# AshishKumar4/FlaxDiff

Measured on AMD Instinct MI355X. Metric: train images/sec/node (64x64 uncond EDM UNet, bs=256), higher is better.
Workload: dtype bf16; 1 GPU; model=unet_64px_[64,128,256,512]_res2_heads4, global_batch=256, resolution=64, parallelism=dp1, schedule=EDM + KarrasPredictionTransform(sigma_data=0.5)

## Files before the change

### flaxdiff_amd/ops/hip/conv2d_halo_v2.hip

```cpp
#include <torch/extension.h>
#include <ATen/hip/HIPContext.h>
#include "common.h"
#include "host_util.h"

typedef __bf16 bf16v8h __attribute__((ext_vector_type(8)));

#define HV2_NTH 256
#define HV2_BK 64

union HBF8 { bf16v8h v; ushort u[8]; uint4 q; };

__device__ __forceinline__ void hv2_glds16(const ushort* src, ushort* dst) {
    __builtin_amdgcn_global_load_lds(
        (const __attribute__((address_space(1))) void*)src,
        (__attribute__((address_space(3))) void*)dst, 16, 0, 0);
}

struct HaloEpilogue {
    float4 bs[2][2][2];
    uint4 av[2][2][2], bv[2][2][2];

    __device__ __forceinline__ void load_bias(const float* __restrict__ bias,
                                              const int nl) {
        #pragma unroll
        for (int fn = 0; fn < 2; ++fn) {
            #pragma unroll
            for (int p = 0; p < 2; ++p) {
                const float4* b = reinterpret_cast<const float4*>(
                    bias + nl + fn * 32 + p * 16);
                bs[fn][p][0] = b[0];
                bs[fn][p][1] = b[1];
            }
        }
    }

    __device__ __forceinline__ void load_adds(const ushort* __restrict__ addp,
                                              const ushort* __restrict__ baddp,
                                              const long m0, const int nl,
                                              const long RW, const int Cout,
                                              const long M) {
        #pragma unroll
        for (int fm = 0; fm < 2; ++fm) {
            const long m = m0 + fm * 32;
            const long mc = m < M ? m : M - 1;
            if (addp) {
                const ushort* a = addp + mc * Cout + nl;
                #pragma unroll
                for (int fn = 0; fn < 2; ++fn) {
                    #pragma unroll
                    for (int p = 0; p < 2; ++p)
                        av[fm][fn][p] = *reinterpret_cast<const uint4*>(
                            a + fn * 32 + p * 16);
                }
            }
            if (baddp) {
                const ushort* b = baddp
                    + (long)((unsigned)mc / (unsigned)RW) * Cout + nl;
                #pragma unroll
                for (int fn = 0; fn < 2; ++fn) {
                    #pragma unroll
                    for (int p = 0; p < 2; ++p)
                        bv[fm][fn][p] = *reinterpret_cast<const uint4*>(
                            b + fn * 32 + p * 16);
                }
            }
        }
    }

    static __device__ __forceinline__ void add_bf8(float (&v)[8], const uint4 u) {
        const uint w[4] = {u.x, u.y, u.z, u.w};
        #pragma unroll
        for (int i = 0; i < 4; ++i) {
            v[2 * i] += __uint_as_float(w[i] << 16);
            v[2 * i + 1] += __uint_as_float(w[i] & 0xffff0000u);
        }
    }

    __device__ __forceinline__ void finish(const f32x16 (&acc)[2][2],
                                           const bool has_bias,
                                           const bool has_add,
                                           const bool has_badd,
                                           ushort* __restrict__ Y,
                                           const long m0, const int nl,
                                           const int Cout, const long M) const {
        #pragma unroll
        for (int fm = 0; fm < 2; ++fm) {
            const long m = m0 + fm * 32;
            ushort* yrow = Y + m * Cout + nl;
            #pragma unroll
            for (int fn = 0; fn < 2; ++fn) {
                #pragma unroll
                for (int p = 0; p < 2; ++p) {
                    float v[8];
                    #pragma unroll
                    for (int j = 0; j < 4; ++j) {
                        const auto r = __builtin_amdgcn_permlane32_swap(
                            __float_as_uint(acc[fn][fm][(2 * p) * 4 + j]),
                            __float_as_uint(acc[fn][fm][(2 * p + 1) * 4 + j]),
                            false, false);
                        v[j] = __uint_as_float(r[0]);
                        v[4 + j] = __uint_as_float(r[1]);
                    }
                    if (has_bias) {
                        const float4 b0 = bs[fn][p][0], b1 = bs[fn][p][1];
                        v[0] += b0.x; v[1] += b0.y; v[2] += b0.z; v[3] += b0.w;
                        v[4] += b1.x; v[5] += b1.y; v[6] += b1.z; v[7] += b1.w;
                    }
                    if (has_add) add_bf8(v, av[fm][fn][p]);
                    if (has_badd) add_bf8(v, bv[fm][fn][p]);
                    uint4 pk;
                    pk.x = f2bf(v[0]) | ((uint)f2bf(v[1]) << 16);
                    pk.y = f2bf(v[2]) | ((uint)f2bf(v[3]) << 16);
                    pk.z = f2bf(v[4]) | ((uint)f2bf(v[5]) << 16);
                    pk.w = f2bf(v[6]) | ((uint)f2bf(v[7]) << 16);
                    if (m < M)
                        *reinterpret_cast<uint4*>(yrow + fn * 32 + p * 16) = pk;
                }
            }
        }
    }
};

template <bool TRANSPOSED, int BMT, int BNT, int W, bool UP = false>
__global__ __launch_bounds__(HV2_NTH, 2)
void conv2d_halo_v2_kernel(
        const ushort* __restrict__ X,
        const ushort* __restrict__ Wt,
        const float* __restrict__ bias,
        const ushort* __restrict__ addp,
        const ushort* __restrict__ baddp,
        ushort* __restrict__ Y,
        const int Bn, const int R,
        const int Cin, const int Cout,
        const long M) {
    constexpr int RPT = BMT / W;
    constexpr int NSLOT = RPT + 2;
    constexpr int NROW_H = NSLOT * (W + 2);
    constexpr int ZR = NROW_H;
    constexpr int WB0 = NROW_H + 3;
    constexpr int NW = BNT / 32;
    constexpr int NHC = (NSLOT * W / 8 + 3) / 4;
    constexpr int WMW = BMT / 64;

    extern __shared__ __attribute__((aligned(16))) ushort hlds[];
    const int tid = threadIdx.x;
    const int lane = tid & 63;
    const int wid = tid >> 6;
    const int wn = wid / WMW;
    const int wm = wid % WMW;
    const int half = lane >> 5;
    const int l31 = lane & 31;

    const long m_base = (long)blockIdx.x * BMT;
    const int n_base = blockIdx.y * BNT;
    const long grow0 = m_base / W;
    const long BH = (long)Bn * R;
    const int ksl = Cin / HV2_BK;

    const int n_wave = n_base + wn * 64;
    const bool wave_live = n_wave < Cout;
    const int nl = n_wave + half * 8;
    const long m0 = m_base + wm * 64 + l31;
    HaloEpilogue epi;
    if (bias && wave_live) epi.load_bias(bias, nl);

    auto issue_halo = [&](int ci0) {
        #pragma unroll
        for (int i = 0; i < NHC; ++i) {
            int q = wid + i * 4;
            const int qmax = NSLOT * W / 8 - 1;
            q = q > qmax ? qmax : q;
            const int slot = q / (W / 8);
            const int c = q % (W / 8);
            long g = grow0 + slot - 1;
            g = g < 0 ? 0 : (g >= BH ? BH - 1 : g);
            const int pos0 = c * 8;
            const int rowbase = slot * (W + 2) + 1 + pos0;
            const int pix = pos0 + (lane >> 3);
            const int key = (rowbase + (lane >> 3)) & 7;
            const ushort* s;
            if (UP) {
                const int b = (int)(g / R);
                const int r = (int)(g - (long)b * R);
                const long gs = (long)b * (R >> 1) + (r >> 1);
                s = X + (gs * (W >> 1) + (pix >> 1)) * (long)Cin + ci0
                  + (((lane & 7) ^ key) << 3);
            } else {
                s = X + (g * W + pix) * (long)Cin + ci0
                  + (((lane & 7) ^ key) << 3);
            }
            hv2_glds16(s, hlds + rowbase * 64);
        }
    };
    auto issue_w = [&](int flat) {
        const int tap = flat % 9;
        const int ci0 = (flat / 9) * HV2_BK;
        const ushort* wslab = Wt + (long)tap * Cout * Cin;
        const int buf = (WB0 + (flat % 3) * BNT) * 64;
        #pragma unroll
        for (int i = 0; i < NW; ++i) {
            const int row0 = (wid + i * 4) * 8;
            const int r8 = lane >> 3;
            const int key = ((row0 + r8) & 7);
            int co = n_base + row0 + r8;
            co = co < Cout ? co : Cout - 1;
            const ushort* s = wslab + (long)co * Cin + ci0
                            + (((lane & 7) ^ key) << 3);
            hv2_glds16(s, hlds + buf + row0 * 64);
        }
    };

    f32x16 acc[2][2] = {};
    const int nflat = 9 * ksl;

    issue_halo(0);
    issue_w(0);
    issue_w(1);

    for (int i = tid; i < 3 * 64; i += HV2_NTH)
        hlds[ZR * 64 + i] = 0;
    for (int i = tid; i < NSLOT * 2 * 64; i += HV2_NTH) {
        const int sl = i >> 7;
        const int e = (i >> 6) & 1;
        hlds[(sl * (W + 2) + (e ? (W + 1) : 0)) * 64 + (i & 63)] = 0;
    }

    int brow[2][3];
    #pragma unroll
    for (int fm = 0; fm < 2; ++fm) {
        const long m = m0 + fm * 32;
        const unsigned mc = (unsigned)(m < M ? m : M - 1);
        const int ow = (int)(mc % W);
        const unsigned grow = mc / W;
        const int orow = (int)(grow % (unsigned)R);
        #pragma unroll
        for (int dr = -1; dr <= 1; ++dr) {
            if (m >= M || orow + dr < 0 || orow + dr >= R) {
                brow[fm][dr + 1] = ZR + 1;
            } else {
                const int slot = (int)(grow - (unsigned)grow0) + dr + 1;
                brow[fm][dr + 1] = slot * (W + 2) + ow + 1;
            }
        }
    }

    auto tap_step = [&](const int flat, const bool last) {
        const int tap = flat % 9;
        const int sci = flat / 9;
        if (last || (tap == 0 && sci > 0)) {
            asm volatile("s_waitcnt vmcnt(0) lgkmcnt(0)" ::: "memory");
        } else {
            asm volatile("s_waitcnt vmcnt(%0) lgkmcnt(0)" :: "i"(NW) : "memory");
        }
        __builtin_amdgcn_s_barrier();
        if (last) {
            if (wave_live)
                epi.load_adds(addp, baddp, m0, nl, (long)R * W, Cout, M);
        } else if (flat + 2 < nflat) {
            issue_w(flat + 2);
        }

        const int r = tap / 3, s = tap % 3;
        const int dr = TRANSPOSED ? (1 - r) : (r - 1);
        const int ds = TRANSPOSED ? (1 - s) : (s - 1);
        const int wbuf = (WB0 + (flat % 3) * BNT) * 64;
        const int ar0 = wn * 64 + l31;
        const int ar1 = ar0 + 32;
        const int br0 = brow[0][dr + 1] + ds;
        const int br1 = brow[1][dr + 1] + ds;
        #pragma unroll
        for (int kk = 0; kk < HV2_BK / 16; ++kk) {
            const int k0 = kk * 16 + half * 8;
            const int ch = k0 >> 3;
            bf16v8h a0 = reinterpret_cast<const HBF8*>(
                hlds + wbuf + ar0 * 64 + ((ch ^ (ar0 & 7)) << 3))->v;
            bf16v8h a1 = reinterpret_cast<const HBF8*>(
                hlds + wbuf + ar1 * 64 + ((ch ^ (ar1 & 7)) << 3))->v;
            bf16v8h b0 = reinterpret_cast<const HBF8*>(
                hlds + br0 * 64 + ((ch ^ (br0 & 7)) << 3))->v;
            bf16v8h b1 = reinterpret_cast<const HBF8*>(
                hlds + br1 * 64 + ((ch ^ (br1 & 7)) << 3))->v;
            acc[0][0] = __builtin_amdgcn_mfma_f32_32x32x16_bf16(a0, b0, acc[0][0], 0, 0, 0);
            acc[0][1] = __builtin_amdgcn_mfma_f32_32x32x16_bf16(a0, b1, acc[0][1], 0, 0, 0);
            acc[1][0] = __builtin_amdgcn_mfma_f32_32x32x16_bf16(a1, b0, acc[1][0], 0, 0, 0);
            acc[1][1] = __builtin_amdgcn_mfma_f32_32x32x16_bf16(a1, b1, acc[1][1], 0, 0, 0);
        }
        if (!last && tap == 8) {
            __builtin_amdgcn_s_barrier();
            issue_halo((sci + 1) * HV2_BK);
        }
    };
    for (int flat = 0; flat < nflat - 1; ++flat)
        tap_step(flat, false);
    tap_step(nflat - 1, true);

    if (wave_live)
        epi.finish(acc, bias != nullptr, addp != nullptr, baddp != nullptr,
                   Y, m0, nl, Cout, M);
}

template <int BMT, int BNT, int W>
static size_t hv2_smem() {
    constexpr int NROW = (BMT / W + 2) * (W + 2) + 3 + 3 * BNT;
    return (size_t)NROW * 64 * sizeof(ushort);
}

bool conv2d_halo_v2_launch(const void* x, const void* wt, const float* bias,
                           const ushort* addp, const ushort* baddp,
                           void* y, bool transposed,
                           int B, int R, int W, int Cin, int Cout, long M,
                           hipStream_t stream, bool upsample) {
    FD_FLUSH_STALE();
    if (Cin % 64 || Cout % 64) return false;
    if (M >= (1L << 31)) return false;
    if (W != 8 && W != 16 && W != 32 && W != 64) return false;
    int bmt = (Cout <= 64) ? 256 : 128;
    static const bool w64_256tile = std::getenv("FD_HALO_W64_128TILE") == nullptr;
    if (bmt == 128 && W == 64) {
        if (!w64_256tile) {
            if (Cin / HV2_BK < 2) return false;
        } else {
            bmt = 256;
        }
    }
    const int bnt = 128 * 128 / bmt;
    if (bmt % W) return false;
    if (M % W) return false;

    if (upsample && ((R & 1) || (W & 1))) return false;

    dim3 grid((unsigned)((M + bmt - 1) / bmt), (unsigned)((Cout + bnt - 1) / bnt));
    const int mode = upsample ? 2 : (transposed ? 1 : 0);
    #define HV2_KEY(MODE_, BMT_, W_) (((MODE_) << 16) | ((BMT_) << 7) | (W_))
    #define HV2_CASE(MODE_, BMT_, W_)                                          \
        case HV2_KEY(MODE_, BMT_, W_):                                         \
            fd_launch_lds<conv2d_halo_v2_kernel<(MODE_ == 1), BMT_,            \
                                                128 * 128 / BMT_, W_,          \
                                                (MODE_ == 2)>>(                \
                grid, dim3(HV2_NTH), hv2_smem<BMT_, 128 * 128 / BMT_, W_>(),   \
                stream, (const ushort*)x, (const ushort*)wt, bias, addp,       \
                baddp, (ushort*)y, B, R, Cin, Cout, M);                        \
            break;
    #define HV2_TILE(MODE_, BMT_)                                              \
        HV2_CASE(MODE_, BMT_, 8) HV2_CASE(MODE_, BMT_, 16)                     \
        HV2_CASE(MODE_, BMT_, 32) HV2_CASE(MODE_, BMT_, 64)
    switch (HV2_KEY(mode, bmt, W)) {
        HV2_TILE(0, 128) HV2_TILE(0, 256)
        HV2_TILE(1, 128) HV2_TILE(1, 256)
        HV2_TILE(2, 128) HV2_TILE(2, 256)
        default: return false;
    }
    #undef HV2_TILE
    #undef HV2_CASE
    #undef HV2_KEY
    FD_CHECK_LAUNCH();
    return true;
}
```

### flaxdiff_amd/ops/hip/gemm_bf16.hip

```cpp
#include <torch/extension.h>
#include <ATen/hip/HIPContext.h>
#include "common.h"
#include "host_util.h"

typedef __bf16 bf16v8m __attribute__((ext_vector_type(8)));
typedef __attribute__((__vector_size__(4 * sizeof(__bf16)))) __bf16 bf16x4m;

#define GM_NTH 256
#define GM_BK 64

union MBF8 { bf16v8m v; ushort u[8]; uint4 q; ushort4 h4[2]; };

__device__ __forceinline__ void gm_glds16(const ushort* src, ushort* dst) {
    __builtin_amdgcn_global_load_lds(
        (const __attribute__((address_space(1))) void*)src,
        (__attribute__((address_space(3))) void*)dst, 16, 0, 0);
}

__device__ __forceinline__ bf16x4m gm_tr(const ushort* p) {
    return __builtin_amdgcn_ds_read_tr16_b64_v4bf16(
        (__attribute__((address_space(3))) bf16x4m*)p);
}

template <bool BT, int BMT, int BNT, int LOOK, bool XSPLIT = false>
__global__ __launch_bounds__(GM_NTH, 2)
void gemm_bf16_kernel(const ushort* __restrict__ X,
                      const ushort* __restrict__ W,
                      const float* __restrict__ bias,
                      const ushort* __restrict__ addp,
                      ushort* __restrict__ Y,
                      const long M, const int N, const int K,
                      const long mt_lo_stride,
                      const ushort* __restrict__ X2,
                      const int Ka) {
    constexpr int WMW = BMT / 64;
    constexpr int XTILE = BMT * GM_BK;
    constexpr int KP = (BNT == 128) ? 68 : 64;
    constexpr int WTILE = BT ? (BNT * GM_BK) : ((BNT / 16) * KP * 16);
    constexpr int DBUF = LOOK + 1;
    constexpr int NGX = BMT / 32;
    constexpr int NGW = BNT / 32;
    constexpr int NG = NGX + NGW;

    extern __shared__ __attribute__((aligned(16))) ushort gmlds[];
    ushort* Xr = gmlds;
    ushort* Wr = gmlds + DBUF * XTILE;

    const int tid = threadIdx.x;
    const int lane = tid & 63;
    const int wid = tid >> 6;
    const int wn = wid / WMW;
    const int wm = wid % WMW;
    const int half = lane >> 5;
    const int l31 = lane & 31;
    const int n_base = blockIdx.y * BNT;
    const int ksl = K / GM_BK;

    const long mt0 = (long)blockIdx.x * mt_lo_stride;
    const long mtiles = (M + BMT - 1) / BMT;
    const long mt1 = (mt0 + mt_lo_stride < mtiles) ? mt0 + mt_lo_stride : mtiles;
    const int nsteps = (int)(mt1 - mt0) * ksl;
    if (nsteps <= 0) return;

    auto issue = [&](int f) {
        const int fc = f >= nsteps ? nsteps - 1 : f;
        const long mb = (mt0 + fc / ksl) * BMT;
        const int k0 = (fc % ksl) * GM_BK;
        const int buf = fc % DBUF;
        ushort* xd = Xr + buf * XTILE;
        const ushort* xs = X + k0;
        int xstride = K;
        if (XSPLIT) {
            const bool second = k0 >= Ka;
            xs = second ? X2 + (k0 - Ka) : X + k0;
            xstride = second ? K - Ka : Ka;
        }
        #pragma unroll
        for (int i = 0; i < NGX; ++i) {
            const int row0 = (wid + i * 4) * 8;
            const int r8 = lane >> 3;
            long m = mb + row0 + r8;
            m = m < M ? m : M - 1;
            const int key = (row0 + r8) & 7;
            gm_glds16(xs + m * xstride + (((lane & 7) ^ key) << 3),
                      xd + row0 * GM_BK);
        }
        ushort* wd = Wr + buf * WTILE;
        if (BT) {
            #pragma unroll
            for (int i = 0; i < NGW; ++i) {
                const int row0 = (wid + i * 4) * 8;
                const int r8 = lane >> 3;
                int n = n_base + row0 + r8;
                n = n < N ? n : N - 1;
                const int key = (row0 + r8) & 7;
                gm_glds16(W + (long)n * K + k0 + (((lane & 7) ^ key) << 3),
                          wd + row0 * GM_BK);
            }
        } else {
            #pragma unroll
            for (int i = 0; i < NGW; ++i) {
                const int pi = wid + i * 4;
                const int p = pi >> 1;
                const int kr0 = (pi & 1) * 32;
                int nc = n_base + p * 16 + (lane & 1) * 8;
                if (nc + 8 > N) nc = N - 8;
                gm_glds16(W + (long)(k0 + kr0 + (lane >> 1)) * N + nc,
                          wd + p * KP * 16 + kr0 * 16);
            }
        }
    };

    #pragma unroll
    for (int l = 0; l < LOOK; ++l) issue(l);

    const int ltr = ((lane >> 4) & 1) * KP * 16 + ((lane >> 5) << 3) * 16
                  + (lane & 15) * 4;

    constexpr int NFN = 2;
    f32x16 acc[NFN][2] = {};

    long cur_mt = mt0;
    for (int f = 0; f < nsteps; ++f) {
        asm volatile("s_waitcnt vmcnt(%0)" :: "i"((LOOK - 1) * NG) : "memory");
        __builtin_amdgcn_s_barrier();
        issue(f + LOOK);
        const int buf = f % DBUF;
        const ushort* Xb = Xr + buf * XTILE;
        const ushort* Wb = Wr + buf * WTILE;

        #pragma unroll
        for (int kk = 0; kk < GM_BK / 16; ++kk) {
            const int k0 = kk * 16 + half * 8;
            const int ch = k0 >> 3;
            MBF8 a0, a1;
            if (BT) {
                const int ar0 = wn * 64 + l31;
                a0 = *reinterpret_cast<const MBF8*>(
                    Wb + ar0 * GM_BK + ((ch ^ (ar0 & 7)) << 3));
                if (NFN == 2) {
                    const int ar1 = ar0 + 32;
                    a1 = *reinterpret_cast<const MBF8*>(
                        Wb + ar1 * GM_BK + ((ch ^ (ar1 & 7)) << 3));
                }
            } else {
                const ushort* ap = Wb + wn * 4 * KP * 16 + ltr + kk * 16 * 16;
                bf16x4m t0 = gm_tr(ap), t1 = gm_tr(ap + 64);
                a0.h4[0] = *reinterpret_cast<ushort4*>(&t0);
                a0.h4[1] = *reinterpret_cast<ushort4*>(&t1);
                if (NFN == 2) {
                    const ushort* ap2 = ap + 2 * KP * 16;
                    bf16x4m t2 = gm_tr(ap2), t3 = gm_tr(ap2 + 64);
                    a1.h4[0] = *reinterpret_cast<ushort4*>(&t2);
                    a1.h4[1] = *reinterpret_cast<ushort4*>(&t3);
                }
            }
            const int br0 = wm * 64 + l31;
            const int br1 = br0 + 32;
            const bf16v8m b0 = reinterpret_cast<const MBF8*>(
                Xb + br0 * GM_BK + ((ch ^ (br0 & 7)) << 3))->v;
            const bf16v8m b1 = reinterpret_cast<const MBF8*>(
                Xb + br1 * GM_BK + ((ch ^ (br1 & 7)) << 3))->v;
            acc[0][0] = __builtin_amdgcn_mfma_f32_32x32x16_bf16(a0.v, b0, acc[0][0], 0, 0, 0);
            acc[0][1] = __builtin_amdgcn_mfma_f32_32x32x16_bf16(a0.v, b1, acc[0][1], 0, 0, 0);
            if (NFN == 2) {
                acc[1][0] = __builtin_amdgcn_mfma_f32_32x32x16_bf16(a1.v, b0, acc[1][0], 0, 0, 0);
                acc[1][1] = __builtin_amdgcn_mfma_f32_32x32x16_bf16(a1.v, b1, acc[1][1], 0, 0, 0);
            }
        }

        if ((f % ksl) == ksl - 1) {
            const long m_base = cur_mt * BMT;
            #pragma unroll
            for (int fm = 0; fm < 2; ++fm) {
                const long m = m_base + wm * 64 + fm * 32 + l31;
                if (m < M) {
                    ushort* yrow = Y + m * N;
                    #pragma unroll
                    for (int fn = 0; fn < NFN; ++fn) {
                        #pragma unroll
                        for (int qq = 0; qq < 4; ++qq) {
                            const int n0 = n_base + wn * 64 + fn * 32 + qq * 8
                                         + half * 4;
                            if (n0 >= N) continue;
                            float v0 = acc[fn][fm][qq * 4 + 0];
                            float v1 = acc[fn][fm][qq * 4 + 1];
                            float v2 = acc[fn][fm][qq * 4 + 2];
                            float v3 = acc[fn][fm][qq * 4 + 3];
                            if (bias) {
                                v0 += bias[n0];
                                v1 += (n0 + 1 < N) ? bias[n0 + 1] : 0.f;
                                v2 += (n0 + 2 < N) ? bias[n0 + 2] : 0.f;
                                v3 += (n0 + 3 < N) ? bias[n0 + 3] : 0.f;
                            }
                            if (addp && n0 + 4 <= N) {
                                const ushort4 av = *reinterpret_cast<
                                    const ushort4*>(addp + m * N + n0);
                                v0 += bf2f(av.x); v1 += bf2f(av.y);
                                v2 += bf2f(av.z); v3 += bf2f(av.w);
                            } else if (addp) {
                                for (int j = 0; j < 4 && n0 + j < N; ++j) {
                                    const float av = bf2f(addp[m * N + n0 + j]);
                                    if (j == 0) v0 += av;
                                    else if (j == 1) v1 += av;
                                    else if (j == 2) v2 += av;
                                    else v3 += av;
                                }
                            }
                            if (n0 + 4 <= N) {
                                ushort4 pk;
                                pk.x = f2bf(v0); pk.y = f2bf(v1);
                                pk.z = f2bf(v2); pk.w = f2bf(v3);
                                *reinterpret_cast<ushort4*>(yrow + n0) = pk;
                            } else {
                                const float vs[4] = {v0, v1, v2, v3};
                                for (int j = 0; j < 4 && n0 + j < N; ++j)
                                    yrow[n0 + j] = f2bf(vs[j]);
                            }
                        }
                    }
                }
            }
            #pragma unroll
            for (int a = 0; a < NFN; ++a) {
                acc[a][0] = (f32x16){};
                acc[a][1] = (f32x16){};
            }
            ++cur_mt;
        }
    }
    asm volatile("s_waitcnt vmcnt(0)" ::: "memory");
}

torch::Tensor gemm_fwd(torch::Tensor x, torch::Tensor w, torch::Tensor bias) {
    FD_FLUSH_STALE();
    TORCH_CHECK(x.is_cuda() && x.is_contiguous() && w.is_contiguous());
    TORCH_CHECK(x.scalar_type() == at::kBFloat16 && w.scalar_type() == at::kBFloat16);
    const long M = x.size(0);
    const int K = x.size(1), N = w.size(1);
    TORCH_CHECK(w.size(0) == K && K % GM_BK == 0);
    auto y = torch::empty({M, (long)N}, x.options());
    const float* bias_ptr = nullptr;
    torch::Tensor bias_f;
    if (bias.defined() && bias.numel()) {
        bias_f = bias.to(at::kFloat).contiguous();
        bias_ptr = bias_f.data_ptr<float>();
    }
    const int bmt = (N <= 64) ? 256 : 128;
    const int bnt = 128 * 128 / bmt;
    const long mtiles = (M + bmt - 1) / bmt;
    const int ntiles = (N + bnt - 1) / bnt;
    long bm = std::max<long>(1, std::min<long>(mtiles, 768 / std::max(1, ntiles)));
    const long tpb = (mtiles + bm - 1) / bm;
    bm = (mtiles + tpb - 1) / tpb;
    auto stream = at::hip::getCurrentHIPStream();
    dim3 grid((unsigned)bm, (unsigned)ntiles);
    if (bmt == 256) {
        constexpr size_t smem = 2 * (256 * 64 + 4 * 64 * 16) * sizeof(ushort);
        fd_launch_lds<gemm_bf16_kernel<false, 256, 64, 1>>(grid, dim3(GM_NTH), smem, stream,
                           (const ushort*)x.data_ptr(), (const ushort*)w.data_ptr(),
                           bias_ptr, nullptr, (ushort*)y.data_ptr(), M, N, K, tpb,
                           (const ushort*)nullptr, 0);
    } else {
        constexpr size_t smem = 2 * (128 * 64 + 8 * 68 * 16) * sizeof(ushort);
        fd_launch_lds<gemm_bf16_kernel<false, 128, 128, 1>>(grid, dim3(GM_NTH), smem, stream,
                           (const ushort*)x.data_ptr(), (const ushort*)w.data_ptr(),
                           bias_ptr, nullptr, (ushort*)y.data_ptr(), M, N, K, tpb,
                           (const ushort*)nullptr, 0);
    }
    FD_CHECK_LAUNCH();
    return y;
}

torch::Tensor gemm_dx(torch::Tensor dy, torch::Tensor w) {
    FD_FLUSH_STALE();
    TORCH_CHECK(dy.is_cuda() && dy.is_contiguous() && w.is_contiguous());
    const long M = dy.size(0);
    const int N = dy.size(1), K = w.size(0);
    TORCH_CHECK(w.size(1) == N && N % GM_BK == 0);
    auto dx = torch::empty({M, (long)K}, dy.options());
    const int bmt = (K <= 64) ? 256 : 128;
    const int bnt = 128 * 128 / bmt;
    const long mtiles = (M + bmt - 1) / bmt;
    const int ntiles = (K + bnt - 1) / bnt;
    long bm = std::max<long>(1, std::min<long>(mtiles, 768 / std::max(1, ntiles)));
    const long tpb = (mtiles + bm - 1) / bm;
    bm = (mtiles + tpb - 1) / tpb;
    auto stream = at::hip::getCurrentHIPStream();
    dim3 grid((unsigned)bm, (unsigned)ntiles);
    if (bmt == 256) {
        constexpr size_t smem = 2 * (256 * 64 + 64 * 64) * sizeof(ushort);
        fd_launch_lds<gemm_bf16_kernel<true, 256, 64, 1>>(grid, dim3(GM_NTH), smem, stream,
                           (const ushort*)dy.data_ptr(), (const ushort*)w.data_ptr(),
                           nullptr, nullptr, (ushort*)dx.data_ptr(), M, K, N, tpb,
                           (const ushort*)nullptr, 0);
    } else {
        constexpr size_t smem = 2 * (128 * 64 + 128 * 64) * sizeof(ushort);
        fd_launch_lds<gemm_bf16_kernel<true, 128, 128, 1>>(grid, dim3(GM_NTH), smem, stream,
                           (const ushort*)dy.data_ptr(), (const ushort*)w.data_ptr(),
                           nullptr, nullptr, (ushort*)dx.data_ptr(), M, K, N, tpb,
                           (const ushort*)nullptr, 0);
    }
    FD_CHECK_LAUNCH();
    return dx;
}

torch::Tensor gemm_nt(torch::Tensor x, torch::Tensor wt, torch::Tensor bias,
                      torch::Tensor addt, c10::optional<torch::Tensor> x2) {
    FD_FLUSH_STALE();
    TORCH_CHECK(x.is_cuda() && x.is_contiguous() && wt.is_contiguous());
    const long M = x.size(0);
    const bool split = fd_has(x2);
    const int Ka = x.size(1);
    const ushort* x2_ptr = nullptr;
    if (split) {
        TORCH_CHECK(x2->is_cuda() && x2->device() == x.device() &&
                    x2->is_contiguous() && x2->dim() == 2 && x2->size(0) == M &&
                    x2->scalar_type() == at::kBFloat16 &&
                    x.scalar_type() == at::kBFloat16 &&
                    Ka % GM_BK == 0 && x2->size(1) % GM_BK == 0,
                    "gemm_nt: x2 must be bf16 [M, Kb] with Ka, Kb % 64 == 0");
        x2_ptr = (const ushort*)x2->data_ptr();
    }
    const int K = Ka + (split ? (int)x2->size(1) : 0), N = wt.size(0);
    TORCH_CHECK(wt.size(1) == K && K % GM_BK == 0);
    auto y = torch::empty({M, (long)N}, x.options());
    const float* bias_ptr = nullptr;
    torch::Tensor bias_f;
    if (bias.defined() && bias.numel()) {
        bias_f = bias.to(at::kFloat).contiguous();
        bias_ptr = bias_f.data_ptr<float>();
    }
    const ushort* add_ptr = nullptr;
    if (addt.defined() && addt.numel()) {
        TORCH_CHECK(addt.is_contiguous() && addt.numel() == M * N &&
                    addt.scalar_type() == at::kBFloat16,
                    "gemm_nt add tensor must be bf16 [M, N]");
        add_ptr = (const ushort*)addt.data_ptr();
    }
    const int bmt = (N <= 64) ? 256 : 128;
    const int bnt = 128 * 128 / bmt;
    const long mtiles = (M + bmt - 1) / bmt;
    const int ntiles = (N + bnt - 1) / bnt;
    long bm = std::max<long>(1, std::min<long>(mtiles, 768 / std::max(1, ntiles)));
    const long tpb = (mtiles + bm - 1) / bm;
    bm = (mtiles + tpb - 1) / tpb;
    auto stream = at::hip::getCurrentHIPStream();
    dim3 grid((unsigned)bm, (unsigned)ntiles);
    #define GM_NT_LAUNCH(BMT_, BNT_, SPLIT_)                                   \
        fd_launch_lds<gemm_bf16_kernel<true, BMT_, BNT_, 1, SPLIT_>>(          \
            grid, dim3(GM_NTH),                                                \
            (size_t)2 * (BMT_ * 64 + BNT_ * 64) * sizeof(ushort), stream,      \
            (const ushort*)x.data_ptr(), (const ushort*)wt.data_ptr(),         \
            bias_ptr, add_ptr, (ushort*)y.data_ptr(), M, N, K, tpb,            \
            x2_ptr, Ka)
    if (bmt == 256) {
        if (split) GM_NT_LAUNCH(256, 64, true);
        else GM_NT_LAUNCH(256, 64, false);
    } else {
        if (split) GM_NT_LAUNCH(128, 128, true);
        else GM_NT_LAUNCH(128, 128, false);
    }
    #undef GM_NT_LAUNCH
    FD_CHECK_LAUNCH();
    return y;
}

__global__ void transpose_shadows_kernel(const ushort* __restrict__ src_base,
                                         ushort* __restrict__ dst_base,
                                         const int* __restrict__ tiles,
                                         const int ntiles2) {
    __shared__ ushort tsm[64][65];
    for (int t = blockIdx.x; t < ntiles2; t += gridDim.x) {
        const int* rec = tiles + (long)t * 4;
        const long soff = (unsigned)rec[0];
        const long doff = (unsigned)rec[1];
        const int N = rec[2];
        const int K = rec[3];
        const int lane = threadIdx.x & 63;
        const int w = threadIdx.x >> 6;
        __syncthreads();
        #pragma unroll
        for (int r = 0; r < 16; ++r) {
            const int row = w * 16 + r;
            tsm[row][lane] = src_base[soff + (long)row * N + lane];
        }
        __syncthreads();
        #pragma unroll
        for (int r = 0; r < 16; ++r) {
            const int row = w * 16 + r;
            dst_base[doff + (long)row * K + lane] = tsm[lane][row];
        }
    }
}

void transpose_shadows(torch::Tensor src_flat, torch::Tensor dst_flat,
                       torch::Tensor tiles) {
    FD_FLUSH_STALE();
    TORCH_CHECK(src_flat.is_cuda() && tiles.scalar_type() == at::kInt);
    const int n = tiles.size(0);
    if (!n) return;
    auto stream = at::hip::getCurrentHIPStream();
    const int blocks = std::min(n, 2048);
    hipLaunchKernelGGL(transpose_shadows_kernel, dim3(blocks), dim3(256), 0,
                       stream, (const ushort*)src_flat.data_ptr(),
                       (ushort*)dst_flat.data_ptr(), tiles.data_ptr<int>(), n);
    FD_CHECK_LAUNCH();
}
```

Baseline: 6230 images/s.

## Unify LDS swizzle keys with compile-time conflict proofs and share the vectorized MFMA epilogue

Moves the XOR chunk swizzle into a shared lds_swizzle header. The halo conv now adds a per-slot key delta so B-fragment reads across halo rows avoid LDS bank conflicts, and constexpr static_asserts check that reads stay conflict-free for each tile shape and width. The GEMM kernel gains a FAST template path that reuses the halo conv's permlane-based epilogue, with bias preloaded and add tensors prefetched before the final k-step, so stores are 16-byte vectorized. This adds register pressure for the prefetched epilogue data and more template variants to compile.

Result: faster. 6381 images/s, median of 6 (+2.4%).

```diff
diff --git a/flaxdiff_amd/ops/hip/conv2d_halo_v2.hip b/flaxdiff_amd/ops/hip/conv2d_halo_v2.hip
--- a/flaxdiff_amd/ops/hip/conv2d_halo_v2.hip
+++ b/flaxdiff_amd/ops/hip/conv2d_halo_v2.hip
@@ -2,6 +2,8 @@
 #include <ATen/hip/HIPContext.h>
 #include "common.h"
 #include "host_util.h"
+#include "lds_swizzle.h"
+#include "mfma_epilogue.h"
 
 typedef __bf16 bf16v8h __attribute__((ext_vector_type(8)));
 
@@ -15,111 +17,6 @@
         (const __attribute__((address_space(1))) void*)src,
         (__attribute__((address_space(3))) void*)dst, 16, 0, 0);
 }
-
-struct HaloEpilogue {
-    float4 bs[2][2][2];
-    uint4 av[2][2][2], bv[2][2][2];
-
-    __device__ __forceinline__ void load_bias(const float* __restrict__ bias,
-                                              const int nl) {
-        #pragma unroll
-        for (int fn = 0; fn < 2; ++fn) {
-            #pragma unroll
-            for (int p = 0; p < 2; ++p) {
-                const float4* b = reinterpret_cast<const float4*>(
-                    bias + nl + fn * 32 + p * 16);
-                bs[fn][p][0] = b[0];
-                bs[fn][p][1] = b[1];
-            }
-        }
-    }
-
-    __device__ __forceinline__ void load_adds(const ushort* __restrict__ addp,
-                                              const ushort* __restrict__ baddp,
-                                              const long m0, const int nl,
-                                              const long RW, const int Cout,
-                                              const long M) {
-        #pragma unroll
-        for (int fm = 0; fm < 2; ++fm) {
-            const long m = m0 + fm * 32;
-            const long mc = m < M ? m : M - 1;
-            if (addp) {
-                const ushort* a = addp + mc * Cout + nl;
-                #pragma unroll
-                for (int fn = 0; fn < 2; ++fn) {
-                    #pragma unroll
-                    for (int p = 0; p < 2; ++p)
-                        av[fm][fn][p] = *reinterpret_cast<const uint4*>(
-                            a + fn * 32 + p * 16);
-                }
-            }
-            if (baddp) {
-                const ushort* b = baddp
-                    + (long)((unsigned)mc / (unsigned)RW) * Cout + nl;
-                #pragma unroll
-                for (int fn = 0; fn < 2; ++fn) {
-                    #pragma unroll
-                    for (int p = 0; p < 2; ++p)
-                        bv[fm][fn][p] = *reinterpret_cast<const uint4*>(
-                            b + fn * 32 + p * 16);
-                }
-            }
-        }
-    }
-
-    static __device__ __forceinline__ void add_bf8(float (&v)[8], const uint4 u) {
-        const uint w[4] = {u.x, u.y, u.z, u.w};
-        #pragma unroll
-        for (int i = 0; i < 4; ++i) {
-            v[2 * i] += __uint_as_float(w[i] << 16);
-            v[2 * i + 1] += __uint_as_float(w[i] & 0xffff0000u);
-        }
-    }
-
-    __device__ __forceinline__ void finish(const f32x16 (&acc)[2][2],
-                                           const bool has_bias,
-                                           const bool has_add,
-                                           const bool has_badd,
-                                           ushort* __restrict__ Y,
-                                           const long m0, const int nl,
-                                           const int Cout, const long M) const {
-        #pragma unroll
-        for (int fm = 0; fm < 2; ++fm) {
-            const long m = m0 + fm * 32;
-            ushort* yrow = Y + m * Cout + nl;
-            #pragma unroll
-            for (int fn = 0; fn < 2; ++fn) {
-                #pragma unroll
-                for (int p = 0; p < 2; ++p) {
-                    float v[8];
-                    #pragma unroll
-                    for (int j = 0; j < 4; ++j) {
-                        const auto r = __builtin_amdgcn_permlane32_swap(
-                            __float_as_uint(acc[fn][fm][(2 * p) * 4 + j]),
-                            __float_as_uint(acc[fn][fm][(2 * p + 1) * 4 + j]),
-                            false, false);
-                        v[j] = __uint_as_float(r[0]);
-                        v[4 + j] = __uint_as_float(r[1]);
-                    }
-                    if (has_bias) {
-                        const float4 b0 = bs[fn][p][0], b1 = bs[fn][p][1];
-                        v[0] += b0.x; v[1] += b0.y; v[2] += b0.z; v[3] += b0.w;
-                        v[4] += b1.x; v[5] += b1.y; v[6] += b1.z; v[7] += b1.w;
-                    }
-                    if (has_add) add_bf8(v, av[fm][fn][p]);
-                    if (has_badd) add_bf8(v, bv[fm][fn][p]);
-                    uint4 pk;
-                    pk.x = f2bf(v[0]) | ((uint)f2bf(v[1]) << 16);
-                    pk.y = f2bf(v[2]) | ((uint)f2bf(v[3]) << 16);
-                    pk.z = f2bf(v[4]) | ((uint)f2bf(v[5]) << 16);
-                    pk.w = f2bf(v[6]) | ((uint)f2bf(v[7]) << 16);
-                    if (m < M)
-                        *reinterpret_cast<uint4*>(yrow + fn * 32 + p * 16) = pk;
-                }
-            }
-        }
-    }
-};
 
 template <bool TRANSPOSED, int BMT, int BNT, int W, bool UP = false>
 __global__ __launch_bounds__(HV2_NTH, 2)
@@ -177,7 +74,8 @@
             const int pos0 = c * 8;
             const int rowbase = slot * (W + 2) + 1 + pos0;
             const int pix = pos0 + (lane >> 3);
-            const int key = (rowbase + (lane >> 3)) & 7;
+            const int key = lds_swz::chunk_key(
+                rowbase + (lane >> 3) + lds_swz::halo_key_delta(W) * slot);
             const ushort* s;
             if (UP) {
                 const int b = (int)(g / R);
@@ -201,7 +99,7 @@
         for (int i = 0; i < NW; ++i) {
             const int row0 = (wid + i * 4) * 8;
             const int r8 = lane >> 3;
-            const int key = ((row0 + r8) & 7);
+            const int key = lds_swz::chunk_key(row0 + r8);
             int co = n_base + row0 + r8;
             co = co < Cout ? co : Cout - 1;
             const ushort* s = wslab + (long)co * Cin + ci0
@@ -226,6 +124,7 @@
     }
 
     int brow[2][3];
+    int kd[2];
     #pragma unroll
     for (int fm = 0; fm < 2; ++fm) {
         const long m = m0 + fm * 32;
@@ -233,6 +132,7 @@
         const int ow = (int)(mc % W);
         const unsigned grow = mc / W;
         const int orow = (int)(grow % (unsigned)R);
+        kd[fm] = lds_swz::halo_key_delta(W) * ((int)(grow - (unsigned)grow0) + 1);
         #pragma unroll
         for (int dr = -1; dr <= 1; ++dr) {
             if (m >= M || orow + dr < 0 || orow + dr >= R) {
@@ -268,18 +168,22 @@
         const int ar1 = ar0 + 32;
         const int br0 = brow[0][dr + 1] + ds;
         const int br1 = brow[1][dr + 1] + ds;
+        const int kdr = lds_swz::halo_key_delta(W) * dr;
+        const int ka0 = lds_swz::chunk_key(ar0), ka1 = lds_swz::chunk_key(ar1);
+        const int kb0 = lds_swz::chunk_key(br0 + kd[0] + kdr);
+        const int kb1 = lds_swz::chunk_key(br1 + kd[1] + kdr);
         #pragma unroll
         for (int kk = 0; kk < HV2_BK / 16; ++kk) {
             const int k0 = kk * 16 + half * 8;
             const int ch = k0 >> 3;
             bf16v8h a0 = reinterpret_cast<const HBF8*>(
-                hlds + wbuf + ar0 * 64 + ((ch ^ (ar0 & 7)) << 3))->v;
+                hlds + wbuf + ar0 * 64 + ((ch ^ ka0) << 3))->v;
             bf16v8h a1 = reinterpret_cast<const HBF8*>(
-                hlds + wbuf + ar1 * 64 + ((ch ^ (ar1 & 7)) << 3))->v;
+                hlds + wbuf + ar1 * 64 + ((ch ^ ka1) << 3))->v;
             bf16v8h b0 = reinterpret_cast<const HBF8*>(
-                hlds + br0 * 64 + ((ch ^ (br0 & 7)) << 3))->v;
+                hlds + br0 * 64 + ((ch ^ kb0) << 3))->v;
             bf16v8h b1 = reinterpret_cast<const HBF8*>(
-                hlds + br1 * 64 + ((ch ^ (br1 & 7)) << 3))->v;
+                hlds + br1 * 64 + ((ch ^ kb1) << 3))->v;
             acc[0][0] = __builtin_amdgcn_mfma_f32_32x32x16_bf16(a0, b0, acc[0][0], 0, 0, 0);
             acc[0][1] = __builtin_amdgcn_mfma_f32_32x32x16_bf16(a0, b1, acc[0][1], 0, 0, 0);
             acc[1][0] = __builtin_amdgcn_mfma_f32_32x32x16_bf16(a1, b0, acc[1][0], 0, 0, 0);
diff --git a/flaxdiff_amd/ops/hip/gemm_bf16.hip b/flaxdiff_amd/ops/hip/gemm_bf16.hip
--- a/flaxdiff_amd/ops/hip/gemm_bf16.hip
+++ b/flaxdiff_amd/ops/hip/gemm_bf16.hip
@@ -2,6 +2,9 @@
 #include <ATen/hip/HIPContext.h>
 #include "common.h"
 #include "host_util.h"
+#define LDS_SWZ_NO_HALO_PROOF
+#include "lds_swizzle.h"
+#include "mfma_epilogue.h"
 
 typedef __bf16 bf16v8m __attribute__((ext_vector_type(8)));
 typedef __attribute__((__vector_size__(4 * sizeof(__bf16)))) __bf16 bf16x4m;
@@ -22,7 +25,7 @@
         (__attribute__((address_space(3))) bf16x4m*)p);
 }
 
-template <bool BT, int BMT, int BNT, int LOOK, bool XSPLIT = false>
+template <bool BT, int BMT, int BNT, int LOOK, bool XSPLIT, bool FAST>
 __global__ __launch_bounds__(GM_NTH, 2)
 void gemm_bf16_kernel(const ushort* __restrict__ X,
                       const ushort* __restrict__ W,
@@ -81,7 +84,7 @@
             const int r8 = lane >> 3;
             long m = mb + row0 + r8;
             m = m < M ? m : M - 1;
-            const int key = (row0 + r8) & 7;
+            const int key = lds_swz::chunk_key(row0 + r8);
             gm_glds16(xs + m * xstride + (((lane & 7) ^ key) << 3),
                       xd + row0 * GM_BK);
         }
@@ -93,7 +96,7 @@
                 const int r8 = lane >> 3;
                 int n = n_base + row0 + r8;
                 n = n < N ? n : N - 1;
-                const int key = (row0 + r8) & 7;
+                const int key = lds_swz::chunk_key(row0 + r8);
                 gm_glds16(W + (long)n * K + k0 + (((lane & 7) ^ key) << 3),
                           wd + row0 * GM_BK);
             }
@@ -111,6 +114,12 @@
         }
     };
 
+    const int n_wave = n_base + wn * 64;
+    const bool wave_live = n_wave < N;
+    const int nl = n_wave + half * 8;
+    HaloEpilogue epi;
+    if (FAST && bias && wave_live) epi.load_bias(bias, nl);
+
     #pragma unroll
     for (int l = 0; l < LOOK; ++l) issue(l);
 
@@ -124,6 +133,10 @@
     for (int f = 0; f < nsteps; ++f) {
         asm volatile("s_waitcnt vmcnt(%0)" :: "i"((LOOK - 1) * NG) : "memory");
         __builtin_amdgcn_s_barrier();
+        const bool tile_done = (f % ksl) == ksl - 1;
+        const long m0 = cur_mt * BMT + wm * 64 + l31;
+        if (FAST && tile_done && wave_live && addp)
+            epi.load_adds(addp, nullptr, m0, nl, 1, N, M);
         issue(f + LOOK);
         const int buf = f % DBUF;
         const ushort* Xb = Xr + buf * XTILE;
@@ -137,11 +150,11 @@
             if (BT) {
                 const int ar0 = wn * 64 + l31;
                 a0 = *reinterpret_cast<const MBF8*>(
-                    Wb + ar0 * GM_BK + ((ch ^ (ar0 & 7)) << 3));
+                    Wb + ar0 * GM_BK + ((ch ^ lds_swz::chunk_key(ar0)) << 3));
                 if (NFN == 2) {
                     const int ar1 = ar0 + 32;
                     a1 = *reinterpret_cast<const MBF8*>(
-                        Wb + ar1 * GM_BK + ((ch ^ (ar1 & 7)) << 3));
+                        Wb + ar1 * GM_BK + ((ch ^ lds_swz::chunk_key(ar1)) << 3));
                 }
             } else {
                 const ushort* ap = Wb + wn * 4 * KP * 16 + ltr + kk * 16 * 16;
@@ -158,9 +171,9 @@
             const int br0 = wm * 64 + l31;
             const int br1 = br0 + 32;
             const bf16v8m b0 = reinterpret_cast<const MBF8*>(
-                Xb + br0 * GM_BK + ((ch ^ (br0 & 7)) << 3))->v;
+                Xb + br0 * GM_BK + ((ch ^ lds_swz::chunk_key(br0)) << 3))->v;
             const bf16v8m b1 = reinterpret_cast<const MBF8*>(
-                Xb + br1 * GM_BK + ((ch ^ (br1 & 7)) << 3))->v;
+                Xb + br1 * GM_BK + ((ch ^ lds_swz::chunk_key(br1)) << 3))->v;
             acc[0][0] = __builtin_amdgcn_mfma_f32_32x32x16_bf16(a0.v, b0, acc[0][0], 0, 0, 0);
             acc[0][1] = __builtin_amdgcn_mfma_f32_32x32x16_bf16(a0.v, b1, acc[0][1], 0, 0, 0);
             if (NFN == 2) {
@@ -169,53 +182,59 @@
             }
         }
 
-        if ((f % ksl) == ksl - 1) {
-            const long m_base = cur_mt * BMT;
-            #pragma unroll
-            for (int fm = 0; fm < 2; ++fm) {
-                const long m = m_base + wm * 64 + fm * 32 + l31;
-                if (m < M) {
-                    ushort* yrow = Y + m * N;
-                    #pragma unroll
-                    for (int fn = 0; fn < NFN; ++fn) {
+        if (tile_done) {
+            if (FAST) {
+                if (wave_live)
+                    epi.finish(acc, bias != nullptr, addp != nullptr, false,
+                               Y, m0, nl, N, M);
+            } else {
+                const long m_base = cur_mt * BMT;
+                #pragma unroll
+                for (int fm = 0; fm < 2; ++fm) {
+                    const long m = m_base + wm * 64 + fm * 32 + l31;
+                    if (m < M) {
+                        ushort* yrow = Y + m * N;
                         #pragma unroll
-                        for (int qq = 0; qq < 4; ++qq) {
-                            const int n0 = n_base + wn * 64 + fn * 32 + qq * 8
-                                         + half * 4;
-                            if (n0 >= N) continue;
-                            float v0 = acc[fn][fm][qq * 4 + 0];
-                            float v1 = acc[fn][fm][qq * 4 + 1];
-                            float v2 = acc[fn][fm][qq * 4 + 2];
-                            float v3 = acc[fn][fm][qq * 4 + 3];
-                            if (bias) {
-                                v0 += bias[n0];
-                                v1 += (n0 + 1 < N) ? bias[n0 + 1] : 0.f;
-                                v2 += (n0 + 2 < N) ? bias[n0 + 2] : 0.f;
-                                v3 += (n0 + 3 < N) ? bias[n0 + 3] : 0.f;
-                            }
-                            if (addp && n0 + 4 <= N) {
-                                const ushort4 av = *reinterpret_cast<
-                                    const ushort4*>(addp + m * N + n0);
-                                v0 += bf2f(av.x); v1 += bf2f(av.y);
-                                v2 += bf2f(av.z); v3 += bf2f(av.w);
-                            } else if (addp) {
-                                for (int j = 0; j < 4 && n0 + j < N; ++j) {
-                                    const float av = bf2f(addp[m * N + n0 + j]);
-                                    if (j == 0) v0 += av;
-                                    else if (j == 1) v1 += av;
-                                    else if (j == 2) v2 += av;
-                                    else v3 += av;
+                        for (int fn = 0; fn < NFN; ++fn) {
+                            #pragma unroll
+                            for (int qq = 0; qq < 4; ++qq) {
+                                const int n0 = n_base + wn * 64 + fn * 32 + qq * 8
+                                             + half * 4;
+                                if (n0 >= N) continue;
+                                float v0 = acc[fn][fm][qq * 4 + 0];
+                                float v1 = acc[fn][fm][qq * 4 + 1];
+                                float v2 = acc[fn][fm][qq * 4 + 2];
+                                float v3 = acc[fn][fm][qq * 4 + 3];
+                                if (bias) {
+                                    v0 += bias[n0];
+                                    v1 += (n0 + 1 < N) ? bias[n0 + 1] : 0.f;
+                                    v2 += (n0 + 2 < N) ? bias[n0 + 2] : 0.f;
+                                    v3 += (n0 + 3 < N) ? bias[n0 + 3] : 0.f;
                                 }
-                            }
-                            if (n0 + 4 <= N) {
-                                ushort4 pk;
-                                pk.x = f2bf(v0); pk.y = f2bf(v1);
-                                pk.z = f2bf(v2); pk.w = f2bf(v3);
-                                *reinterpret_cast<ushort4*>(yrow + n0) = pk;
-                            } else {
-                                const float vs[4] = {v0, v1, v2, v3};
-                                for (int j = 0; j < 4 && n0 + j < N; ++j)
-                                    yrow[n0 + j] = f2bf(vs[j]);
+                                if (addp && n0 + 4 <= N) {
+                                    const ushort4 av = *reinterpret_cast<
+                                        const ushort4*>(addp + m * N + n0);
+                                    v0 += bf2f(av.x); v1 += bf2f(av.y);
+                                    v2 += bf2f(av.z); v3 += bf2f(av.w);
+                                } else if (addp) {
+                                    for (int j = 0; j < 4 && n0 + j < N; ++j) {
+                                        const float av = bf2f(addp[m * N + n0 + j]);
+                                        if (j == 0) v0 += av;
+                                        else if (j == 1) v1 += av;
+                                        else if (j == 2) v2 += av;
+                                        else v3 += av;
+                                    }
+                                }
+                                if (n0 + 4 <= N) {
+                                    ushort4 pk;
+                                    pk.x = f2bf(v0); pk.y = f2bf(v1);
+                                    pk.z = f2bf(v2); pk.w = f2bf(v3);
+                                    *reinterpret_cast<ushort4*>(yrow + n0) = pk;
+                                } else {
+                                    const float vs[4] = {v0, v1, v2, v3};
+                                    for (int j = 0; j < 4 && n0 + j < N; ++j)
+                                        yrow[n0 + j] = f2bf(vs[j]);
+                                }
                             }
                         }
                     }
@@ -230,6 +249,17 @@
         }
     }
     asm volatile("s_waitcnt vmcnt(0)" ::: "memory");
+}
+
+template <bool BT, int BMT, int BNT, bool XSPLIT, typename... Args>
+static void gm_launch(const bool fast, dim3 grid, size_t smem,
+                      hipStream_t stream, Args... args) {
+    if (fast)
+        fd_launch_lds<gemm_bf16_kernel<BT, BMT, BNT, 1, XSPLIT, true>>(
+            grid, dim3(GM_NTH), smem, stream, args...);
+    else
+        fd_launch_lds<gemm_bf16_kernel<BT, BMT, BNT, 1, XSPLIT, false>>(
+            grid, dim3(GM_NTH), smem, stream, args...);
 }
 
 torch::Tensor gemm_fwd(torch::Tensor x, torch::Tensor w, torch::Tensor bias) {
@@ -257,13 +287,13 @@
     dim3 grid((unsigned)bm, (unsigned)ntiles);
     if (bmt == 256) {
         constexpr size_t smem = 2 * (256 * 64 + 4 * 64 * 16) * sizeof(ushort);
-        fd_launch_lds<gemm_bf16_kernel<false, 256, 64, 1>>(grid, dim3(GM_NTH), smem, stream,
+        gm_launch<false, 256, 64, false>(N % 64 == 0, grid, smem, stream,
                            (const ushort*)x.data_ptr(), (const ushort*)w.data_ptr(),
                            bias_ptr, nullptr, (ushort*)y.data_ptr(), M, N, K, tpb,
                            (const ushort*)nullptr, 0);
     } else {
         constexpr size_t smem = 2 * (128 * 64 + 8 * 68 * 16) * sizeof(ushort);
-        fd_launch_lds<gemm_bf16_kernel<false, 128, 128, 1>>(grid, dim3(GM_NTH), smem, stream,
+        gm_launch<false, 128, 128, false>(N % 64 == 0, grid, smem, stream,
                            (const ushort*)x.data_ptr(), (const ushort*)w.data_ptr(),
                            bias_ptr, nullptr, (ushort*)y.data_ptr(), M, N, K, tpb,
                            (const ushort*)nullptr, 0);
@@ -290,13 +320,13 @@
     dim3 grid((unsigned)bm, (unsigned)ntiles);
     if (bmt == 256) {
         constexpr size_t smem = 2 * (256 * 64 + 64 * 64) * sizeof(ushort);
-        fd_launch_lds<gemm_bf16_kernel<true, 256, 64, 1>>(grid, dim3(GM_NTH), smem, stream,
+        gm_launch<true, 256, 64, false>(K % 64 == 0, grid, smem, stream,
                            (const ushort*)dy.data_ptr(), (const ushort*)w.data_ptr(),
                            nullptr, nullptr, (ushort*)dx.data_ptr(), M, K, N, tpb,
                            (const ushort*)nullptr, 0);
     } else {
         constexpr size_t smem = 2 * (128 * 64 + 128 * 64) * sizeof(ushort);
-        fd_launch_lds<gemm_bf16_kernel<true, 128, 128, 1>>(grid, dim3(GM_NTH), smem, stream,
+        gm_launch<true, 128, 128, false>(K % 64 == 0, grid, smem, stream,
                            (const ushort*)dy.data_ptr(), (const ushort*)w.data_ptr(),
                            nullptr, nullptr, (ushort*)dx.data_ptr(), M, K, N, tpb,
                            (const ushort*)nullptr, 0);
@@ -348,8 +378,8 @@
     auto stream = at::hip::getCurrentHIPStream();
     dim3 grid((unsigned)bm, (unsigned)ntiles);
     #define GM_NT_LAUNCH(BMT_, BNT_, SPLIT_)                                   \
-        fd_launch_lds<gemm_bf16_kernel<true, BMT_, BNT_, 1, SPLIT_>>(          \
-            grid, dim3(GM_NTH),                                                \
+        gm_launch<true, BMT_, BNT_, SPLIT_>(                                   \
+            N % 64 == 0, grid,                                                 \
             (size_t)2 * (BMT_ * 64 + BNT_ * 64) * sizeof(ushort), stream,      \
             (const ushort*)x.data_ptr(), (const ushort*)wt.data_ptr(),         \
             bias_ptr, add_ptr, (ushort*)y.data_ptr(), M, N, K, tpb,            \
diff --git a/flaxdiff_amd/ops/hip/lds_swizzle.h b/flaxdiff_amd/ops/hip/lds_swizzle.h
--- /dev/null
+++ b/flaxdiff_amd/ops/hip/lds_swizzle.h
@@ -0,0 +1,186 @@
+#pragma once
+
+#if defined(__HIPCC__)
+#define LDS_SWZ_HD __host__ __device__
+#else
+#define LDS_SWZ_HD
+#endif
+
+namespace lds_swz {
+
+LDS_SWZ_HD constexpr int chunk_key(const int krow) { return (krow >> 1) & 7; }
+
+LDS_SWZ_HD constexpr int halo_key_pitch(const int W) {
+    return W >= 32 ? W + 2 : (W == 16 ? 32 : 24);
+}
+LDS_SWZ_HD constexpr int halo_key_delta(const int W) {
+    return halo_key_pitch(W) - (W + 2);
+}
+LDS_SWZ_HD constexpr int halo_row(const int W, const int slot, const int pos) {
+    return slot * (W + 2) + pos;
+}
+LDS_SWZ_HD constexpr int halo_key_row(const int W, const int slot, const int pos) {
+    return halo_row(W, slot, pos) + halo_key_delta(W) * slot;
+}
+
+constexpr int kB128Group[4][16] = {
+    {0, 1, 2, 3, 12, 13, 14, 15, 20, 21, 22, 23, 24, 25, 26, 27},
+    {4, 5, 6, 7, 8, 9, 10, 11, 16, 17, 18, 19, 28, 29, 30, 31},
+    {32, 33, 34, 35, 44, 45, 46, 47, 52, 53, 54, 55, 56, 57, 58, 59},
+    {36, 37, 38, 39, 40, 41, 42, 43, 48, 49, 50, 51, 60, 61, 62, 63}};
+
+constexpr int b128_cycles(const int (&addr)[64]) {
+    int total = 0;
+    for (int g = 0; g < 4; ++g) {
+        int per_slot[16] = {};
+        int worst = 0;
+        for (int i = 0; i < 16; ++i) {
+            const int a = addr[kB128Group[g][i]];
+            bool first = true;
+            for (int j = 0; j < i; ++j)
+                if (addr[kB128Group[g][j]] == a) first = false;
+            if (first && ++per_slot[(a >> 4) & 15] > worst)
+                worst = per_slot[(a >> 4) & 15];
+        }
+        total += worst;
+    }
+    return total;
+}
+
+struct FragRows { int row[32]; int krow[32]; };
+
+constexpr int frag_cycles(const FragRows& f, const int kk) {
+    int addr[64] = {};
+    for (int lane = 0; lane < 64; ++lane) {
+        const int l31 = lane & 31;
+        const int ch = (2 * kk + (lane >> 5)) ^ chunk_key(f.krow[l31]);
+        addr[lane] = f.row[l31] * 128 + ch * 16;
+    }
+    return b128_cycles(addr);
+}
+
+constexpr int frag_cycles_max(const FragRows& f) {
+    int worst = 0;
+    for (int kk = 0; kk < 4; ++kk) {
+        const int c = frag_cycles(f, kk);
+        worst = c > worst ? c : worst;
+    }
+    return worst;
+}
+
+constexpr int tile_read_cycles(const int abs0, const int base) {
+    FragRows f = {};
+    for (int l = 0; l < 32; ++l) {
+        f.row[l] = abs0 + base + l;
+        f.krow[l] = base + l;
+    }
+    return frag_cycles_max(f);
+}
+
+constexpr int tile_cycles_max(const int abs0, const int rows) {
+    int worst = 0;
+    for (int base = 0; base < rows; base += 32) {
+        const int c = tile_read_cycles(abs0, base);
+        worst = c > worst ? c : worst;
+    }
+    return worst;
+}
+
+constexpr int halo_zero_row(const int BMT, const int W) {
+    return (BMT / W + 2) * (W + 2);
+}
+constexpr int halo_wring_row(const int BMT, const int W) {
+    return halo_zero_row(BMT, W) + 3;
+}
+
+constexpr int halo_b_cycles(const int BMT, const int W, const int wm,
+                            const int fm, const int dr, const int ds,
+                            const int zmask) {
+    FragRows f = {};
+    for (int l = 0; l < 32; ++l) {
+        const int m = wm * 64 + fm * 32 + l;
+        const int slot = m / W + dr + 1;
+        const int pos = m % W + 1 + ds;
+        const bool z = (zmask >> (l / W)) & 1;
+        f.row[l] = z ? halo_zero_row(BMT, W) + 1 + ds : halo_row(W, slot, pos);
+        f.krow[l] = f.row[l] + halo_key_delta(W) * slot;
+    }
+    return frag_cycles_max(f);
+}
+
+template <int BMT, int W, int DR, int DS, int ZMASK>
+inline constexpr int halo_b_tap_max = [] {
+    int worst = 0;
+    for (int wm = 0; wm < BMT / 64; ++wm)
+        for (int fm = 0; fm < 2; ++fm) {
+            const int c = halo_b_cycles(BMT, W, wm, fm, DR, DS, ZMASK);
+            worst = c > worst ? c : worst;
+        }
+    return worst;
+}();
+
+template <int BMT, int W, int ZMASK>
+inline constexpr int halo_b_max = [] {
+    int w = 0;
+    #define LDS_SWZ_TAP(DR, DS) \
+        w = halo_b_tap_max<BMT, W, DR, DS, ZMASK> > w \
+            ? halo_b_tap_max<BMT, W, DR, DS, ZMASK> : w;
+    LDS_SWZ_TAP(-1, -1) LDS_SWZ_TAP(-1, 0) LDS_SWZ_TAP(-1, 1)
+    LDS_SWZ_TAP(0, -1) LDS_SWZ_TAP(0, 0) LDS_SWZ_TAP(0, 1)
+    LDS_SWZ_TAP(1, -1) LDS_SWZ_TAP(1, 0) LDS_SWZ_TAP(1, 1)
+    #undef LDS_SWZ_TAP
+    return w;
+}();
+
+template <int BMT, int W, int ZMASK>
+constexpr int halo_b_zero_row_max() {
+    if constexpr (ZMASK == 0) {
+        return 0;
+    } else {
+        constexpr int rest = halo_b_zero_row_max<BMT, W, ZMASK - 1>();
+        return halo_b_max<BMT, W, ZMASK> > rest ? halo_b_max<BMT, W, ZMASK> : rest;
+    }
+}
+
+template <int BMT, int BNT, int W>
+inline constexpr int halo_w_max = [] {
+    int worst = 0;
+    for (int buf = 0; buf < 3; ++buf) {
+        const int c = tile_cycles_max(halo_wring_row(BMT, W) + buf * BNT, BNT);
+        worst = c > worst ? c : worst;
+    }
+    return worst;
+}();
+
+template <int BMT, int BNT>
+inline constexpr int gemm_read_max = [] {
+    int worst = 0;
+    for (int buf = 0; buf < 2; ++buf) {
+        const int x = tile_cycles_max(buf * BMT, BMT);
+        const int w = tile_cycles_max(2 * BMT + buf * BNT, BNT);
+        worst = x > worst ? x : worst;
+        worst = w > worst ? w : worst;
+    }
+    return worst;
+}();
+
+#if !defined(__HIP_DEVICE_COMPILE__) && !defined(LDS_SWZ_NO_HALO_PROOF)
+#define LDS_SWZ_ASSERT_HALO(BMT, BNT, W)                                       \
+    static_assert(halo_w_max<BMT, BNT, W> == 4, "halo weight read conflicts"); \
+    static_assert(halo_b_max<BMT, W, 0> == 4, "halo B read conflicts");
+LDS_SWZ_ASSERT_HALO(256, 64, 64) LDS_SWZ_ASSERT_HALO(128, 128, 64)
+LDS_SWZ_ASSERT_HALO(256, 64, 32) LDS_SWZ_ASSERT_HALO(128, 128, 32)
+LDS_SWZ_ASSERT_HALO(256, 64, 16) LDS_SWZ_ASSERT_HALO(128, 128, 16)
+LDS_SWZ_ASSERT_HALO(256, 64, 8) LDS_SWZ_ASSERT_HALO(128, 128, 8)
+#undef LDS_SWZ_ASSERT_HALO
+static_assert(halo_b_zero_row_max<256, 16, 3>() <= 8 &&
+              halo_b_zero_row_max<128, 16, 3>() <= 8, "W=16 zero-row reads");
+static_assert(halo_b_zero_row_max<256, 8, 15>() <= 8 &&
+              halo_b_zero_row_max<128, 8, 15>() <= 8, "W=8 zero-row reads");
+#endif
+#if !defined(__HIP_DEVICE_COMPILE__)
+static_assert(gemm_read_max<256, 64> == 4 && gemm_read_max<128, 128> == 4,
+              "GEMM fragment read conflicts");
+#endif
+
+}
diff --git a/flaxdiff_amd/ops/hip/mfma_epilogue.h b/flaxdiff_amd/ops/hip/mfma_epilogue.h
--- /dev/null
+++ b/flaxdiff_amd/ops/hip/mfma_epilogue.h
@@ -0,0 +1,106 @@
+#pragma once
+
+struct HaloEpilogue {
+    float4 bs[2][2][2];
+    uint4 av[2][2][2], bv[2][2][2];
+
+    __device__ __forceinline__ void load_bias(const float* __restrict__ bias,
+                                              const int nl) {
+        #pragma unroll
+        for (int fn = 0; fn < 2; ++fn) {
+            #pragma unroll
+            for (int p = 0; p < 2; ++p) {
+                const float4* b = reinterpret_cast<const float4*>(
+                    bias + nl + fn * 32 + p * 16);
+                bs[fn][p][0] = b[0];
+                bs[fn][p][1] = b[1];
+            }
+        }
+    }
+
+    __device__ __forceinline__ void load_adds(const ushort* __restrict__ addp,
+                                              const ushort* __restrict__ baddp,
+                                              const long m0, const int nl,
+                                              const long RW, const int Cout,
+                                              const long M) {
+        #pragma unroll
+        for (int fm = 0; fm < 2; ++fm) {
+            const long m = m0 + fm * 32;
+            const long mc = m < M ? m : M - 1;
+            if (addp) {
+                const ushort* a = addp + mc * Cout + nl;
+                #pragma unroll
+                for (int fn = 0; fn < 2; ++fn) {
+                    #pragma unroll
+                    for (int p = 0; p < 2; ++p)
+                        av[fm][fn][p] = *reinterpret_cast<const uint4*>(
+                            a + fn * 32 + p * 16);
+                }
+            }
+            if (baddp) {
+                const ushort* b = baddp
+                    + (long)((unsigned)mc / (unsigned)RW) * Cout + nl;
+                #pragma unroll
+                for (int fn = 0; fn < 2; ++fn) {
+                    #pragma unroll
+                    for (int p = 0; p < 2; ++p)
+                        bv[fm][fn][p] = *reinterpret_cast<const uint4*>(
+                            b + fn * 32 + p * 16);
+                }
+            }
+        }
+    }
+
+    static __device__ __forceinline__ void add_bf8(float (&v)[8], const uint4 u) {
+        const uint w[4] = {u.x, u.y, u.z, u.w};
+        #pragma unroll
+        for (int i = 0; i < 4; ++i) {
+            v[2 * i] += __uint_as_float(w[i] << 16);
+            v[2 * i + 1] += __uint_as_float(w[i] & 0xffff0000u);
+        }
+    }
+
+    __device__ __forceinline__ void finish(const f32x16 (&acc)[2][2],
+                                           const bool has_bias,
+                                           const bool has_add,
+                                           const bool has_badd,
+                                           ushort* __restrict__ Y,
+                                           const long m0, const int nl,
+                                           const int Cout, const long M) const {
+        #pragma unroll
+        for (int fm = 0; fm < 2; ++fm) {
+            const long m = m0 + fm * 32;
+            ushort* yrow = Y + m * Cout + nl;
+            #pragma unroll
+            for (int fn = 0; fn < 2; ++fn) {
+                #pragma unroll
+                for (int p = 0; p < 2; ++p) {
+                    float v[8];
+                    #pragma unroll
+                    for (int j = 0; j < 4; ++j) {
+                        const auto r = __builtin_amdgcn_permlane32_swap(
+                            __float_as_uint(acc[fn][fm][(2 * p) * 4 + j]),
+                            __float_as_uint(acc[fn][fm][(2 * p + 1) * 4 + j]),
+                            false, false);
+                        v[j] = __uint_as_float(r[0]);
+                        v[4 + j] = __uint_as_float(r[1]);
+                    }
+                    if (has_bias) {
+                        const float4 b0 = bs[fn][p][0], b1 = bs[fn][p][1];
+                        v[0] += b0.x; v[1] += b0.y; v[2] += b0.z; v[3] += b0.w;
+                        v[4] += b1.x; v[5] += b1.y; v[6] += b1.z; v[7] += b1.w;
+                    }
+                    if (has_add) add_bf8(v, av[fm][fn][p]);
+                    if (has_badd) add_bf8(v, bv[fm][fn][p]);
+                    uint4 pk;
+                    pk.x = f2bf(v[0]) | ((uint)f2bf(v[1]) << 16);
+                    pk.y = f2bf(v[2]) | ((uint)f2bf(v[3]) << 16);
+                    pk.z = f2bf(v[4]) | ((uint)f2bf(v[5]) << 16);
+                    pk.w = f2bf(v[6]) | ((uint)f2bf(v[7]) << 16);
+                    if (m < M)
+                        *reinterpret_cast<uint4*>(yrow + fn * 32 + p * 16) = pk;
+                }
+            }
+        }
+    }
+};
```
